# natir/yacrd

Hardware: AMD Instinct MI355X
Metric: reads_per_sec_classified (higher is better)
Workload: dtype u32

## Files before the change

yacrd_amd/csrc/screen_reg.h:

```cpp
#pragma once
#include "device_common.h"
#include "wave_ops.h"

namespace yk {

#ifndef YK_SCREEN_WINDOW
#define YK_SCREEN_WINDOW 32
#endif
constexpr int kScreenWindow = YK_SCREEN_WINDOW;
constexpr int kScreenTabWords = (64 / 16) * (16 + 2 * kScreenWindow) * 4;
template <int WPB, int WORDS = kScreenTabWords>
__device__ __forceinline__ u32 *wave_screen_scratch()
{
    __shared__ __attribute__((aligned(16))) u32 s_tab[WPB][WORDS];
    return s_tab[threadIdx.x >> 6];
}

template <int LANES>
__device__ __forceinline__ bool group_any(u64 ballot)
{
    if (LANES == 64) return ballot != 0;
    return ((u32)(ballot >> (lane_id() & (u32)(64 - LANES))) & (u32)((1ull << (LANES & 63)) - 1ull)) != 0u;
}

struct HealthyRead {
    u32 a, b;
    i32 F, G;
};
#ifndef YK_SCREEN_SLIDES
#define YK_SCREEN_SLIDES 4
#endif
constexpr int kScreenSlides = YK_SCREEN_SLIDES;

template <int LANES, int WPB, bool SLID = false, int TABW = kScreenTabWords>
__device__ __forceinline__ bool healthy_screen(const uint4 (&v)[4], const bool (&real0)[4], const bool (&real1)[4],
                                               u32 len, i32 c, u32 pmin, u32 pmax, HealthyRead &hr, u32 P = 0, u32 Q = 0,
                                               u32 emin = 0, u32 smax = 0xFFFFFFFFu)
{
    constexpr int NB = LANES, W = kScreenWindow, NBIN = 2 * W + NB, GROUPS = 64 / LANES, PER = W / LANES,
                  ZPER = NBIN / LANES;
    constexpr u32 kEnd = 1u << 10, kField = kEnd - 1u;
    static_assert(W % LANES == 0 && PER >= 1 && W <= 64, "window bins per lane; a window index has six bits");
    static_assert(NBIN % LANES == 0 && GROUPS * NBIN * 4 <= TABW, "scratch");
    const u32 lane = lane_id(), lig = lane & (u32)(LANES - 1), grp = lane / (u32)LANES;
    u32 *tab = wave_screen_scratch<WPB, TABW>() + grp * (u32)(NBIN * 4);
    uint4 *bins = reinterpret_cast<uint4 *>(tab);
    char *tb = reinterpret_cast<char *>(tab);

    const i32 bits = 32 - (i32)__builtin_clz(len | 1u) - ilog2c(NB) + (len != 0 ? 0 : -1);
    const u32 sh = (u32)max(bits, ilog2c(W));
    const u32 span = pmax - pmin, T = span - (u32)W;

#pragma unroll
    for (int q = 0; q < ZPER; q++) bins[lig + (u32)(LANES * q)] = make_uint4(0u, 0u, 0u, 0u);
    wave_lds_sync();

    const u32 cp = (lig & 3u) * 4u;
    u32 one = 1u, one_end = kEnd;
    if constexpr (!SLID) asm volatile("" : "+v"(one), "+v"(one_end));
    u32 ramp = 0;
    auto count = [&](u32 s, u32 e, bool real) {
        const u32 ds = s - pmin, dx = e - pmin;
        const u32 is = min(ds, (u32)W) + (ds >> sh);
        const u32 ie = (dx >> sh) + __builtin_elementwise_sub_sat(dx, T) + (u32)W;
        if constexpr (SLID) {
            const bool in_ramp = ds >= (u32)W && s < emin;
            ramp += (real && s >= pmin && in_ramp) ? 1u : 0u;
            if (real && s >= pmin && !in_ramp) atomicAdd(reinterpret_cast<u32 *>(tb + ((is << 4) + cp)), one);
            if (real && e <= pmax && !(e > smax && dx <= T)) atomicAdd(reinterpret_cast<u32 *>(tb + ((ie << 4) + cp)), one_end);
        } else if (real) {
            atomicAdd(reinterpret_cast<u32 *>(tb + ((is << 4) + cp)), one);
            atomicAdd(reinterpret_cast<u32 *>(tb + ((ie << 4) + cp)), one_end);
        }
    };
#pragma unroll
    for (int j = 0; j < 4; j++) {
        count(v[j].x, v[j].y, real0[j]);
        count(v[j].z, v[j].w, real1[j]);
    }
    wave_lds_sync();

    u32 f[PER], fw = 0;
#pragma unroll
    for (int q = 0; q < PER; q++) {
        const u32 d = lig * (u32)PER + q;
        const u32 it = min((u32)(2 * W) - d + ((span - d) >> sh), (u32)(NBIN - 1));
        const uint4 h4 = bins[d], t4 = bins[it];
        f[q] = ((h4.x + h4.y + h4.z + h4.w) & kField) | ((t4.x + t4.y + t4.z + t4.w) & (kField << 10));
        fw += f[q];
    }
    const uint4 c4 = bins[(u32)W + lig];
    const u32 fincl = gscan_add<LANES>(fw);
    u32 reached = 0;
    {
        const u32 k1 = (u32)min(c + 1, 0x1FF);
        u32 run = fincl - fw + (SLID ? ((512u - k1 + P) | ((512u - k1 + Q) << 10)) : (512u - k1) * (1u | kEnd));
#pragma unroll
        for (int q = 0; q < PER; q++) {
            run += f[q];
            reached += run & (0x200u | (0x200u << 10));
        }
    }
    const u32 cand = (((u32)PER - ((reached >> 9) & 7u)) << 20) | (((u32)PER - (reached >> 19)) << 26);
    const u32 w = (c4.x + c4.y + c4.z + c4.w) & ((kField << 10) | kField);
    const u32 wincl = gscan_add<LANES>(w | cand);
    const u32 ex = wincl - w;
    const i32 x = (i32)(ex & kField) - (i32)((wincl >> 10) & kField);
    const u32 xm = gscan_min<LANES>((w & kField) != 0u ? (u32)(x + 0x10000) : 0xFFFFFFFFu);
    const i32 F = (i32)(fincl & kField) + (SLID ? (i32)P : 0), G = (i32)(fincl >> 10) + (SLID ? (i32)Q : 0);
    hr.F = F, hr.G = G;
    hr.a = pmin + ((wincl >> 20) & 63u);
    hr.b = pmax - (wincl >> 26);
    i32 open0 = F;
    if constexpr (SLID) open0 += (i32)gscan_add<LANES>(ramp);
    const bool deep = xm == 0xFFFFFFFFu || (i32)(xm - 0x10000u) + open0 > c;
    return deep && F > c && G > c;
}

struct VerdictsToGlobal {
    const SweepArgs &a;
    __device__ __forceinline__ void closed(u32 r, u32 ra, u32 rb, u32 len) const
    {
        if (ra != 0 || rb != len) a.closed[r] = make_uint2(ra, rb);
        else a.counts[r] = 0;
        if (a.prefilter == 2) atomicAdd(&a.ctr->prefiltered, 1u);
    }
    __device__ __forceinline__ void deferred(u32 r) const { a.counts[r] = kDeferredMark; }
};

template <int ITEMS>
struct ReadsKnown {
    u64 o[ITEMS];
    u32 n[ITEMS], len[ITEMS];
};

template <int LANES, int ITEMS, bool WIDE, int WPB = 1, class Sink>
__device__ __forceinline__ void screen_reads(const SweepArgs &a, const u32 (&r)[ITEMS], const bool (&active)[ITEMS], const Sink &sink,
                                             const ReadsKnown<ITEMS> *known = nullptr)
{
    constexpr int K = 16;
    const u32 lane = lane_id(), lig = lane & (u32)(LANES - 1);
    const i32 c = (i32)min(a.cov, 0x3FFFFFFFu);
    u32 n[ITEMS], len[ITEMS];
    u64 o[ITEMS];
#pragma unroll
    for (int t = 0; t < ITEMS; t++) {
        o[t] = 0, n[t] = 0, len[t] = 0;
        if (known) {
            if (active[t]) o[t] = known->o[t], n[t] = known->n[t], len[t] = known->len[t];
        } else if (active[t]) {
            const ulonglong2 oo = load_extent(a.off + r[t]);
            o[t] = oo.x;
            n[t] = (u32)(oo.y - oo.x);
            len[t] = a.len[r[t]];
        }
    }
    uint4 v[ITEMS][K / 4];
#pragma unroll
    for (int t = 0; t < ITEMS; t++) {
        const bool two = n[t] >= 2u;
        const uint2 *src = two ? a.iv + o[t] : reinterpret_cast<const uint2 *>(a.off);
        const u32 last2 = two ? n[t] - 2u : 0u;
#pragma unroll
        for (int j = 0; j < K / 4; j++)
            v[t][j] = load_pair<(ITEMS >= 2)>(src + min(2u * (lig + (u32)LANES * j), last2));
    }
#pragma unroll
    for (int t = 0; t < ITEMS; t++) {
        if (t > 0 && __builtin_amdgcn_ballot_w64(active[t]) == 0) break;
        const u32 len_c = min(len[t], kMaxKeyPos);
        u32 smin = v[t][0].x, emax = v[t][0].y, smax = v[t][0].x;
        i32 tmin = 0x7FFFFFFF;
#pragma unroll
        for (int j = 0; j < K / 4; j++) {
            smin = min(smin, min(v[t][j].x, v[t][j].z));
            smax = max(smax, max(v[t][j].x, v[t][j].z));
            emax = max(emax, max(v[t][j].y, v[t][j].w));
            tmin = min(tmin, min((i32)(v[t][j].y - v[t][j].x), (i32)(v[t][j].w - v[t][j].z)));
        }
        const int last_addr = (int)((lane | (u32)(LANES - 1)) << 2);
        const u32 pmin = (u32)__builtin_amdgcn_ds_bpermute(last_addr, (int)gscan_min<LANES>(smin));
        const u32 pmax = (u32)__builtin_amdgcn_ds_bpermute(last_addr, (int)gscan_max<LANES>(emax));
        const bool irregular = n[t] < 2u || pmax > len_c || smax > kMaxKeyPos || tmin < (i32)kScreenWindow;
        const bool girr = group_any<LANES>(__builtin_amdgcn_ballot_w64(irregular));
        const u32 n_eff = girr ? 0u : n[t];
        bool real0[K / 4], real1[K / 4];
#pragma unroll
        for (int j = 0; j < K / 4; j++) {
            const u32 i0 = 2u * (lig + (u32)LANES * j);
            real0[j] = i0 + 1u < n_eff;
            real1[j] = i0 < n_eff;
        }
        HealthyRead hr;
        bool healthy = healthy_screen<LANES, WPB, false, kScreenTabWords>(v[t], real0, real1, len[t], c, pmin, pmax, hr) && !girr;
        if constexpr (kScreenSlides > 0 && WIDE) {
            auto state_of = [&](bool nd, const HealthyRead &h) {
                return (nd ? 1u : 0u) | ((u32)min(max(h.F, 0), 1023) << 1) | ((u32)min(max(h.G, 0), 1023) << 11);
            };
            u32 st = state_of(!healthy && !girr && (i32)n[t] > c && (hr.F <= 3 * c + 6 || hr.G <= c), hr);
            if (__builtin_amdgcn_ballot_w64((st & 1u) != 0 && lig == (u32)(LANES - 1)) != 0) {
                u32 emin = v[t][0].y, smax2 = v[t][0].x;
#pragma unroll
                for (int j = 0; j < K / 4; j++) {
                    emin = min(emin, min(v[t][j].y, v[t][j].w));
                    smax2 = max(smax2, max(v[t][j].x, v[t][j].z));
                }
                const u32 gemin = (u32)__builtin_amdgcn_ds_bpermute(last_addr, (int)gscan_min<LANES>(emin));
                const u32 room_h = gemin - pmin;
                const u32 gsmax = (u32)__builtin_amdgcn_ds_bpermute(last_addr, (int)gscan_max<LANES>(smax2));
                const u32 room_t = pmax - gsmax;
                u32 ht = 0, PQ = 0;
#pragma unroll 1
                for (int slide = 0; slide < kScreenSlides; slide++) {
                    const u32 g = (u32)__builtin_amdgcn_ds_bpermute(last_addr, (int)st);
                    const bool gneed = (g & 1u) != 0;
                    const u32 gF = (g >> 1) & 1023u, gG = g >> 11;
                    if (gneed && (i32)gF <= c) ht += (u32)kScreenWindow, PQ = (PQ & 0xFFFF0000u) | gF;
                    if (gneed && (i32)gG <= c) ht += (u32)kScreenWindow << 16, PQ = (PQ & 0xFFFFu) | (gG << 16);
                    const u32 h0 = ht & 0xFFFFu, t0 = ht >> 16;
                    const bool go = gneed && room_h >= h0 + (u32)kScreenWindow && room_t >= t0 + (u32)kScreenWindow &&
                                    pmax - pmin >= h0 + t0 + 2u * (u32)kScreenWindow;
                    if (__builtin_amdgcn_ballot_w64(go) == 0) break;
                    bool r0[K / 4], r1[K / 4];
#pragma unroll
                    for (int j = 0; j < K / 4; j++) r0[j] = real0[j] && go, r1[j] = real1[j] && go;
                    wave_lds_sync();
                    HealthyRead h2;
                    const bool ok2 = healthy_screen<LANES, WPB, true, kScreenTabWords>(v[t], r0, r1, len[t], c, pmin + h0, pmax - t0, h2, PQ & 0xFFFFu, PQ >> 16, gemin, gsmax);
                    st = go ? state_of(!ok2 && (h2.F <= c || h2.G <= c), h2) : 0u;
                    if (go) healthy = ok2, hr.a = h2.a, hr.b = h2.b, hr.F = h2.F, hr.G = h2.G;
                }
            }
        }
        if (lig == (u32)(LANES - 1) && active[t]) {
            if (healthy || (!girr && (i32)n[t] <= c)) {
                const u32 ra = (i32)n[t] <= c ? len[t] : hr.a, rb = (i32)n[t] <= c ? len[t] : hr.b;
                sink.closed(r[t], ra, rb, len[t]);
            } else {
                sink.deferred(r[t]);
            }
        }
        if (t + 1 < ITEMS) wave_lds_sync();
    }
}

template <int LANES, int ITEMS, bool WIDE = false>
__device__ __forceinline__ void screen_block(const SweepArgs &a, u32 block)
{
    constexpr u32 GROUPS = 64 / LANES;
    const u32 grp = lane_id() / (u32)LANES;
    const u32 list_n = *a.list_n;
    const u32 idx0 = a.first + block * (u32)ITEMS * GROUPS;
    if (idx0 >= list_n) return;
    u32 r[ITEMS];
    bool active[ITEMS];
#pragma unroll
    for (int t = 0; t < ITEMS; t++) {
        const u32 idx = idx0 + (u32)t * GROUPS + grp;
        active[t] = idx < list_n;
        r[t] = active[t] ? a.list[idx] : 0u;
    }
    screen_reads<LANES, ITEMS, WIDE>(a, r, active, VerdictsToGlobal{a});
}

}
```

yacrd_amd/csrc/sweep_wave.h:

```cpp
#pragma once
#include <type_traits>

#include "device_common.h"
#include "screen_reg.h"
#include "wave_ops.h"

namespace yk {

constexpr u32 kPadKey = 0xFFFFFFFEu;

template <int LANES, int K>
__device__ __forceinline__ void sweep_group_keys(u32 (&x)[K], u32 m, u32 len, i32 c,
                                                 bool active, u32 r, u64 badmask, u64 zmask,
                                                 bool zl_check, const SweepArgs &a,
                                                 const LaneConst &lc)
{
    const u32 lane = lane_id(), lig = lane & (u32)(LANES - 1);
    auto slot_of = [&]() {
        u32 rr = r;
        asm volatile("" : "+v"(rr));
        return a.stage + (a.off[rr] + 2 * (u64)rr);
    };

    bitonic_sort<LANES, K, 2>(x, lc);

    if (zl_check) {
        bool dup = false;
#pragma unroll
        for (int q = 0; q + 1 < K; q++) dup |= x[q] == x[q + 1] && (x[q] & 3u) == 1u && x[q] != 1u;
        const u32 prev = gshift_up1<LANES>(x[K - 1]);
        dup |= lig != 0 && prev == x[0] && (prev & 3u) == 1u && prev != 1u;
        badmask |= __builtin_amdgcn_ballot_w64(dup);
    }
    const bool group_bad = LANES == 64   ? badmask != 0
                           : LANES == 32 ? (u32)(badmask >> (lane & 32u)) != 0
                                         : ((u32)(badmask >> (lane & 48u)) & 0xFFFFu) != 0;

    u32 n_starts = 0;
#pragma unroll
    for (int q = 0; q < K; q++) n_starts += x[q] & 1u;
    const u32 delta = 2u * n_starts - (u32)K;
    const u32 dincl = gscan_add<LANES>(delta);
    const i32 depth_in = (i32)(dincl - delta);

    const u32 tail_base = m - lig * (u32)K;
    const u32 len_key = len > kMaxKeyPos ? 0xFFFFFFFFu : (len << kKeyShift);
    u32 mf_incl, ml_incl, mf_in, ml_in;
    u32 cnt = 0, fb = 0, fe = 0, cand = kNoKey;
    auto passes = [&](auto zl_tag) {
        constexpr bool ZL = decltype(zl_tag)::value;
        u32 mf = 0, ml = 0;
        i32 dd = depth_in;
#pragma unroll
        for (int q = 0; q < K; q++) {
            const u32 key = x[q], bit = key & 1u;
            const bool is_s = bit != 0, gt = dd > c + q;
            ml = (is_s && !gt) ? key : ml;
            if (ZL) mf = (!is_s && gt) ? max(mf, key ^ 2u) : mf;
            else mf = (!is_s && gt) ? key : mf;
            dd += (i32)(bit << 1);
        }
        if (!ZL) mf = mf ? (mf ^ 2u) : 0u;
        mf_incl = gscan_max<LANES>(mf);
        ml_incl = gscan_max<LANES>(ml);
        mf_in = max(gshift_up1<LANES>(mf_incl), kNoFlag);
        ml_in = gshift_up1<LANES>(ml_incl);

        u32 tc = ZL ? mf_in : (mf_in ^ 2u);
        u32 cml = ml_in;
        dd = depth_in;
#pragma unroll
        for (int q = 0; q < K; q++) {
            const u32 key = x[q], bit = key & 1u;
            const bool is_s = bit != 0, gt = dd > c + q;
            const bool fl = !is_s && gt, low = is_s && !gt;
            const bool eff = ZL ? (fl && (key ^ 2u) > tc) : fl;
            const u32 begin = ZL ? (tc ^ 2u) : tc;
            const bool close = eff && cml > begin;
            cnt += close ? 1u : 0u;
            fb = close ? begin : fb;
            fe = close ? cml : fe;
            const bool tail = fl && ((u32)dd == tail_base) && key >= len_key;
            cand = min(cand, tail ? (key >> kKeyShift) : kNoKey);
            tc = eff ? (ZL ? (key ^ 2u) : key) : tc;
            cml = low ? key : cml;
            dd += (i32)(bit << 1);
        }
    };
    if (zmask == 0) passes(std::false_type{});
    else passes(std::true_type{});
    i32 d;

    const bool live = active && !group_bad;
    u32 g_closed = 0;
    if (__builtin_amdgcn_ballot_w64(cnt != 0) != 0) {
        const u32 cincl = gscan_add<LANES>(cnt);
        g_closed = cincl;
        u32 pos = cincl - cnt;
        if (live && cnt == 1) {
            slot_of()[pos] = make_uint2(fb >> kKeyShift, fe >> kKeyShift);
        } else if (live && cnt > 1) {
            uint2 *slot = slot_of();
            u32 tc = mf_in, cml = ml_in;
            d = depth_in;
#pragma unroll
            for (int q = 0; q < K; q++) {
                const u32 key = x[q];
                const bool is_s = (key & 1u) != 0, gt = d > c;
                const bool fl = !is_s && gt, low = is_s && !gt;
                const bool eff = fl && (key ^ 2u) > tc;
                if (eff && cml > (tc ^ 2u))
                    slot[pos++] = make_uint2((tc ^ 2u) >> kKeyShift, cml >> kKeyShift);
                tc = eff ? (key ^ 2u) : tc;
                cml = low ? key : cml;
                d += is_s ? 1 : -1;
            }
        }
    }
    u32 min_ge = kNoKey;
    if (__builtin_amdgcn_ballot_w64(cand != kNoKey) != 0) min_ge = gscan_min<LANES>(cand);
    if (lig == LANES - 1 && active) {
        if (group_bad) {
            a.rej_list[atomicAdd(a.rej_count, 1u)] = r;
            a.counts[r] = 0;
        } else {
            a.counts[r] = finish_read(slot_of(), g_closed, mf_incl ? (mf_incl ^ 2u) : 0u, ml_incl, min_ge, len);
        }
    }
}


constexpr int kFilterTabWords = 304, kFilterKeyWords = 512;
template <int WPB>
__device__ __forceinline__ u32 *wave_filter_scratch()
{
    __shared__ __attribute__((aligned(16))) u32 s_scratch[WPB][kFilterTabWords + kFilterKeyWords];
    return s_scratch[threadIdx.x >> 6];
}

template <int LANES, int K, int WPB>
__device__ __forceinline__ bool prefilter(const u32 (&x)[K], u32 n, u32 len, i32 c, u32 (&y)[K / 2],
                                          u32 &m_out)
{
    static_assert(K == 16, "a lane reads its K/2 = 8 compacted keys as two 16-byte vectors");
    constexpr int NB = LANES, CAP = LANES * K / 2, GROUPS = 64 / LANES;
    static_assert(GROUPS * (NB + 1) * 4 <= kFilterTabWords && GROUPS * CAP <= kFilterKeyWords, "scratch");
    const u32 lane = lane_id(), lig = lane & (u32)(LANES - 1), grp = lane / (u32)LANES;
    u32 *scratch = wave_filter_scratch<WPB>();
    u32 *tab = scratch + grp * (u32)((NB + 1) * 4);
    u32 *keys = scratch + kFilterTabWords + grp * (u32)CAP;
    uint4 *my_bin = reinterpret_cast<uint4 *>(tab) + lig;
    uint4 *my_keys = reinterpret_cast<uint4 *>(keys) + lig * 2u;

    const i32 bits = 32 - (i32)__builtin_clz(len | 1u) - ilog2c(NB) + (len != 0 ? 0 : -1);
    const u32 sh = (u32)max(bits, 0), ksh = sh + kKeyShift;

    *my_bin = make_uint4(0u, 0u, 0u, 0u);
    my_keys[0] = make_uint4(kPadKey, kPadKey, kPadKey, kPadKey);
    my_keys[1] = make_uint4(kPadKey, kPadKey, kPadKey, kPadKey);
    wave_lds_sync();
    u32 *cell0 = tab + (lig & 3u);
    u32 *pad_cell = cell0 + NB * 4;
    u32 *cell[K];
#pragma unroll
    for (int q = 0; q < K; q++) {
        const bool real = lig + (u32)LANES * (q / 2) < n;
        u32 *p = cell0 + (x[q] >> ksh) * 4u;
        cell[q] = real ? p : pad_cell;
        atomicAdd(cell[q], (q & 1) ? 0x10000u : 1u);
    }
    wave_lds_sync();
    const uint4 w4 = *my_bin;
    const u32 w = w4.x + w4.y + w4.z + w4.w;
    const u32 incl = gscan_add<LANES>(w);
    const i32 S = (i32)(w & 0xFFFFu), E = (i32)(w >> 16);
    const i32 cs = (i32)(incl & 0xFFFFu), ce = (i32)(incl >> 16);
    const i32 depth_after = cs - ce, depth_at = depth_after - (S - E);
    const bool safe = (cs - S) - ce > c && lig < (len >> sh);
    const u64 sball = __builtin_amdgcn_ballot_w64(safe);
    if (sball == 0) return false;
    const u64 smask = LANES == 64 ? sball
                                  : (sball >> (lane & (u32)(64 - LANES))) & ((1ull << (LANES & 63)) - 1ull);
    const bool head = safe && (((smask << 1) >> lig) & 1ull) == 0;
    const bool tail = safe && (((smask >> 1) >> lig) & 1ull) == 0;
    const u32 hv = gscan_max<LANES>(head ? (((lig + 1u) << 16) | (u32)depth_at) : 0u);
    const i32 net = tail ? depth_after - (i32)(hv & 0xFFFFu) : 0;
    const u32 nsyn = min((u32)(net < 0 ? -net : net), (u32)CAP + 1u);
    const u32 synkey = (((hv >> 16) - 1u) << ksh) | (net > 0 ? 3u : 0u);

    const u32 mine = safe ? nsyn : (u32)(S + E);
    const u32 rincl = gscan_add<LANES>(mine);
    const u32 m = (u32)__builtin_amdgcn_ds_bpermute((int)((lane | (u32)(LANES - 1)) << 2), (int)rincl);
    if (__builtin_amdgcn_ballot_w64(m > (u32)CAP) != 0) return false;
    const u32 base = rincl - mine;
    {
        uint4 b4;
        b4.x = base;
        b4.y = b4.x + (w4.x & 0xFFFFu) + (w4.x >> 16);
        b4.z = b4.y + (w4.y & 0xFFFFu) + (w4.y >> 16);
        b4.w = b4.z + (w4.z & 0xFFFFu) + (w4.z >> 16);
        *my_bin = safe ? make_uint4(CAP, CAP, CAP, CAP) : b4;
        if (lig < 4u) tab[NB * 4 + lig] = (u32)CAP;
    }
#pragma unroll 1
    for (u32 t = 0; t < nsyn; t++) keys[base + t] = synkey;
    wave_lds_sync();
#pragma unroll
    for (int q0 = 0; q0 < K; q0 += 8) {
        u32 pos[8];
#pragma unroll
        for (int q = 0; q < 8; q++) pos[q] = atomicAdd(cell[q0 + q], 1u);
#pragma unroll
        for (int q = 0; q < 8; q++) {
            if (pos[q] < (u32)CAP) keys[pos[q]] = x[q0 + q];
        }
    }
    wave_lds_sync();
    const uint4 lo = my_keys[0], hi = my_keys[1];
    y[0] = lo.x, y[1] = lo.y, y[2] = lo.z, y[3] = lo.w;
    y[4] = hi.x, y[5] = hi.y, y[6] = hi.z, y[7] = hi.w;
    m_out = m;
    return true;
}

template <int LANES, int K, int WPB = 4>
__device__ __forceinline__ void sweep_group_read(const uint2 *__restrict__ iv, u32 n, u32 len,
                                                 u32 cov, bool active, u32 r,
                                                 const SweepArgs &a, const LaneConst &lc)
{
    const u32 lane = lane_id(), lig = lane & (u32)(LANES - 1);
    const i32 c = (i32)min(cov, 0x3FFFFFFFu);

    u32 x[K];
    u32 bad = 0, nz = 0;
    bool plain;
    {
        const uint2 *src = n ? iv : reinterpret_cast<const uint2 *>(a.off);
        const u32 last = n ? n - 1u : 0u;
        uint2 v[K / 2];
#pragma unroll
        for (int j = 0; j < K / 2; j++) v[j] = src[min(lig + (u32)LANES * j, last)];
        const u32 len_c = min(len, kMaxKeyPos);
        u32 irregular = 0;
#pragma unroll
        for (int j = 0; j < K / 2; j++) {
            const bool real = lig + (u32)LANES * j < n;
            irregular |= (real && (v[j].x >= v[j].y || v[j].y > len_c)) ? 1u : 0u;
            x[2 * j] = real ? ((v[j].x << kKeyShift) | 3u) : kPadKey;
            x[2 * j + 1] = real ? (v[j].y << kKeyShift) : kPadKey;
        }
        plain = __builtin_amdgcn_ballot_w64(irregular != 0) == 0;
        if (!plain) {
#pragma unroll
            for (int j = 0; j < K / 2; j++) {
                u32 ks, ke, b = 0, z = 0;
                make_event_keys(v[j], ks, ke, b, z);
                const bool real = lig + (u32)LANES * j < n;
                x[2 * j] = real ? ks : kPadKey;
                x[2 * j + 1] = real ? ke : kPadKey;
                bad |= real ? b : 0u;
                nz += real ? z : 0u;
            }
        }
    }
    const u64 badmask = __builtin_amdgcn_ballot_w64(bad != 0);
    const u64 zmask = __builtin_amdgcn_ballot_w64(nz != 0);
    if (LANES == 64 && badmask != 0) {
        if (lig == LANES - 1 && active) {
            a.rej_list[atomicAdd(a.rej_count, 1u)] = r;
            a.counts[r] = 0;
        }
        return;
    }
    const bool zl_check = (zmask & (zmask - 1)) != 0 || __builtin_amdgcn_ballot_w64(nz > 2) != 0;

    if constexpr (K == 16) {
        if (a.prefilter && plain) {
            u32 y[K / 2], mf;
            if (prefilter<LANES, K, WPB>(x, n, len, c, y, mf)) {
                if (a.prefilter == 2 && lig == 0 && active) atomicAdd(&a.ctr->prefiltered, 1u);
                sweep_group_keys<LANES, K / 2>(y, mf, len, c, active, r, badmask, zmask, zl_check, a, lc);
                return;
            }
        }
    }
    sweep_group_keys<LANES, K>(x, 2 * n, len, c, active, r, badmask, zmask, zl_check, a, lc);
}

template <int LANES, int K, int WPB = 4>
__device__ __forceinline__ void sweep_group_block(const SweepArgs &a, u32 block)
{
    const u32 lane = lane_id();
    const LaneConst lc = make_lane_const(lane);

    constexpr u32 GROUPS = 64 / LANES;
    const u32 list_n = *a.list_n;
    const u32 wave = block * (u32)WPB + (threadIdx.x >> 6);
    if (a.first + wave * GROUPS >= list_n) return;
    const u32 idx = a.first + wave * GROUPS + lane / (u32)LANES;
    const bool active = idx < list_n;
    u32 r = 0, n = 0, len = 0;
    u64 o = 0;
    if (active) {
        r = a.list[idx];
        o = a.off[r];
        n = (u32)(a.off[r + 1] - o);
        len = a.len[r];
    }
    sweep_group_read<LANES, K, WPB>(a.iv + o, n, len, a.cov, active, r, a, lc);
}

template <int LANES, int K>
__global__ __launch_bounds__(256) void sweep_group_kernel(SweepArgs a)
{
    sweep_group_block<LANES, K>(a, blockIdx.x);
}

template <int LANES, int K>
inline void launch_sweep_group(const SweepArgs &sa, u32 n_reads, hipStream_t stream)
{
    constexpr u32 per_block = 4u * (64 / LANES);
    const u32 grid = (n_reads + per_block - 1) / per_block;
    hipLaunchKernelGGL((sweep_group_kernel<LANES, K>), dim3(grid ? grid : 1), dim3(256), 0, stream, sa);
}

#ifndef YK_DEFER_OCC
#define YK_DEFER_OCC 6
#endif
constexpr int kFusedWaves = 4, kDeferWaves = 1, kDeferOcc = YK_DEFER_OCC;
static_assert(kDeferWaves == 1, "screen_block indexes list entries by workgroup: one wavefront each");
struct FusedArgs {
    SweepArgs base;
    u32 n_entries;
    u32 cls[5];
    u32 block_end[5];
    u32 first[5];
    const u32 *list[5];
    const u32 *list_n[5];
};

template <bool DEFER, int WPB, int ITEMS = 1, bool WIDE = false>
__device__ __forceinline__ void sweep_small_fused_body(const FusedArgs &f)
{
    u32 g = blockIdx.x;
    {
        const u32 nb = gridDim.x, x = g & 7u, q = nb >> 3, rem = nb & 7u;
        g = x * q + min(x, rem) + (g >> 3);
    }
    u32 e = 0, first = 0;
    while (e + 1 < f.n_entries && g >= f.block_end[e]) {
        first = f.block_end[e];
        e++;
    }
    SweepArgs a = f.base;
    a.list = f.list[e];
    a.list_n = f.list_n[e];
    a.first = f.first[e];
    const u32 b = g - first;
    switch (f.cls[e]) {
    case CLS_R2: sweep_group_block<16, 2, WPB>(a, b); break;
    case CLS_R4: sweep_group_block<16, 4, WPB>(a, b); break;
    case CLS_R8: sweep_group_block<16, 8, WPB>(a, b); break;
    case CLS_R16:
        if constexpr (DEFER) screen_block<16, ITEMS, WIDE>(a, b);
        else sweep_group_block<16, 16, WPB>(a, b);
        break;
    default:
        if constexpr (DEFER) screen_block<32, ITEMS, WIDE>(a, b);
        else sweep_group_block<32, 16, WPB>(a, b);
        break;
    }
}
__global__ __launch_bounds__(64 * kDeferWaves, kDeferOcc) void sweep_small_fused_defer_kernel(FusedArgs f)
{
    sweep_small_fused_body<true, kDeferWaves>(f);
}
__global__ __launch_bounds__(64 * kDeferWaves, kDeferOcc) void sweep_small_fused_defer_wide_kernel(FusedArgs f)
{
    sweep_small_fused_body<true, kDeferWaves, 1, true>(f);
}
#ifndef YK_DEFER2_OCC
#define YK_DEFER2_OCC YK_DEFER_OCC
#endif
__global__ __launch_bounds__(64, YK_DEFER2_OCC) void sweep_small_fused_defer2_kernel(FusedArgs f)
{
    sweep_small_fused_body<true, 1, 2>(f);
}
__global__ __launch_bounds__(64 * kFusedWaves, 5) void sweep_small_fused_kernel(FusedArgs f)
{
    sweep_small_fused_body<false, kFusedWaves>(f);
}

inline u32 sweep_group_reads_per_block(int cls, int waves = 4)
{
    return ((cls <= CLS_R16) ? 4u : (cls == CLS_H16) ? 2u : 1u) * (u32)waves;
}

}
```

Measured before the change: 2.921 billion.

## Screen 32-interval reads with 16-lane groups holding two bins per lane

Makes healthy_screen generic in bin count and interval pairs per lane, so a 16-lane group can cover 32 bins with two bins per lane and scan over them locally. In the defer2 (two-item, non-wide) kernel, the default-class reads now go through 16-lane groups processing one read with K=32 intervals, instead of 32-lane groups with two items. The scratch table grows to fit the larger bin count. The aim is to screen four reads per wave instead of two. The cost is more per-lane work, more registers and more LDS per wave.

```diff
diff --git a/yacrd_amd/csrc/screen_reg.h b/yacrd_amd/csrc/screen_reg.h
--- a/yacrd_amd/csrc/screen_reg.h
+++ b/yacrd_amd/csrc/screen_reg.h
@@ -9,6 +9,7 @@
 #endif
 constexpr int kScreenWindow = YK_SCREEN_WINDOW;
 constexpr int kScreenTabWords = (64 / 16) * (16 + 2 * kScreenWindow) * 4;
+constexpr int kScreenTabWordsRows = (64 / 16) * (32 + 2 * kScreenWindow) * 4;
 template <int WPB, int WORDS = kScreenTabWords>
 __device__ __forceinline__ u32 *wave_screen_scratch()
 {
@@ -32,16 +33,17 @@
 #endif
 constexpr int kScreenSlides = YK_SCREEN_SLIDES;
 
-template <int LANES, int WPB, bool SLID = false, int TABW = kScreenTabWords>
-__device__ __forceinline__ bool healthy_screen(const uint4 (&v)[4], const bool (&real0)[4], const bool (&real1)[4],
+template <int LANES, int WPB, bool SLID = false, int TABW = kScreenTabWords, int NB = LANES, int PAIRS = 4>
+__device__ __forceinline__ bool healthy_screen(const uint4 (&v)[PAIRS], const bool (&real0)[PAIRS], const bool (&real1)[PAIRS],
                                                u32 len, i32 c, u32 pmin, u32 pmax, HealthyRead &hr, u32 P = 0, u32 Q = 0,
                                                u32 emin = 0, u32 smax = 0xFFFFFFFFu)
 {
-    constexpr int NB = LANES, W = kScreenWindow, NBIN = 2 * W + NB, GROUPS = 64 / LANES, PER = W / LANES,
-                  ZPER = NBIN / LANES;
+    constexpr int W = kScreenWindow, NBIN = 2 * W + NB, GROUPS = 64 / LANES, PER = W / LANES, ZPER = NBIN / LANES,
+                  CPL = NB / LANES;
     constexpr u32 kEnd = 1u << 10, kField = kEnd - 1u;
     static_assert(W % LANES == 0 && PER >= 1 && W <= 64, "window bins per lane; a window index has six bits");
-    static_assert(NBIN % LANES == 0 && GROUPS * NBIN * 4 <= TABW, "scratch");
+    static_assert(NB % LANES == 0 && NBIN % LANES == 0 && GROUPS * NBIN * 4 <= TABW, "scratch");
+    static_assert(PAIRS * 2 * LANES <= 256, "a counter field has ten bits");
     const u32 lane = lane_id(), lig = lane & (u32)(LANES - 1), grp = lane / (u32)LANES;
     u32 *tab = wave_screen_scratch<WPB, TABW>() + grp * (u32)(NBIN * 4);
     uint4 *bins = reinterpret_cast<uint4 *>(tab);
@@ -74,7 +76,7 @@
         }
     };
 #pragma unroll
-    for (int j = 0; j < 4; j++) {
+    for (int j = 0; j < PAIRS; j++) {
         count(v[j].x, v[j].y, real0[j]);
         count(v[j].z, v[j].w, real1[j]);
     }
@@ -89,7 +91,13 @@
         f[q] = ((h4.x + h4.y + h4.z + h4.w) & kField) | ((t4.x + t4.y + t4.z + t4.w) & (kField << 10));
         fw += f[q];
     }
-    const uint4 c4 = bins[(u32)W + lig];
+    u32 wb[CPL], w = 0;
+#pragma unroll
+    for (int q = 0; q < CPL; q++) {
+        const uint4 c4 = bins[(u32)W + lig * (u32)CPL + q];
+        wb[q] = (c4.x + c4.y + c4.z + c4.w) & ((kField << 10) | kField);
+        w += wb[q];
+    }
     const u32 fincl = gscan_add<LANES>(fw);
     u32 reached = 0;
     {
@@ -102,11 +110,16 @@
         }
     }
     const u32 cand = (((u32)PER - ((reached >> 9) & 7u)) << 20) | (((u32)PER - (reached >> 19)) << 26);
-    const u32 w = (c4.x + c4.y + c4.z + c4.w) & ((kField << 10) | kField);
     const u32 wincl = gscan_add<LANES>(w | cand);
-    const u32 ex = wincl - w;
-    const i32 x = (i32)(ex & kField) - (i32)((wincl >> 10) & kField);
-    const u32 xm = gscan_min<LANES>((w & kField) != 0u ? (u32)(x + 0x10000) : 0xFFFFFFFFu);
+    u32 run = wincl - w, xl = 0xFFFFFFFFu;
+#pragma unroll
+    for (int q = 0; q < CPL; q++) {
+        const u32 ex = run;
+        run += wb[q];
+        const i32 x = (i32)(ex & kField) - (i32)((run >> 10) & kField);
+        xl = min(xl, (wb[q] & kField) != 0u ? (u32)(x + 0x10000) : 0xFFFFFFFFu);
+    }
+    const u32 xm = gscan_min<LANES>(xl);
     const i32 F = (i32)(fincl & kField) + (SLID ? (i32)P : 0), G = (i32)(fincl >> 10) + (SLID ? (i32)Q : 0);
     hr.F = F, hr.G = G;
     hr.a = pmin + ((wincl >> 20) & 63u);
@@ -134,11 +147,12 @@
     u32 n[ITEMS], len[ITEMS];
 };
 
-template <int LANES, int ITEMS, bool WIDE, int WPB = 1, class Sink>
+template <int LANES, int ITEMS, bool WIDE, int WPB = 1, int K = 16, int NB = LANES, bool NT = (ITEMS >= 2),
+          int TABW = kScreenTabWords, class Sink>
 __device__ __forceinline__ void screen_reads(const SweepArgs &a, const u32 (&r)[ITEMS], const bool (&active)[ITEMS], const Sink &sink,
                                              const ReadsKnown<ITEMS> *known = nullptr)
 {
-    constexpr int K = 16;
+    static_assert(K % 4 == 0, "a lane takes its intervals in pairs");
     const u32 lane = lane_id(), lig = lane & (u32)(LANES - 1);
     const i32 c = (i32)min(a.cov, 0x3FFFFFFFu);
     u32 n[ITEMS], len[ITEMS];
@@ -163,7 +177,7 @@
         const u32 last2 = two ? n[t] - 2u : 0u;
 #pragma unroll
         for (int j = 0; j < K / 4; j++)
-            v[t][j] = load_pair<(ITEMS >= 2)>(src + min(2u * (lig + (u32)LANES * j), last2));
+            v[t][j] = load_pair<NT>(src + min(2u * (lig + (u32)LANES * j), last2));
     }
 #pragma unroll
     for (int t = 0; t < ITEMS; t++) {
@@ -192,7 +206,7 @@
             real1[j] = i0 < n_eff;
         }
         HealthyRead hr;
-        bool healthy = healthy_screen<LANES, WPB, false, kScreenTabWords>(v[t], real0, real1, len[t], c, pmin, pmax, hr) && !girr;
+        bool healthy = healthy_screen<LANES, WPB, false, TABW, NB>(v[t], real0, real1, len[t], c, pmin, pmax, hr) && !girr;
         if constexpr (kScreenSlides > 0 && WIDE) {
             auto state_of = [&](bool nd, const HealthyRead &h) {
                 return (nd ? 1u : 0u) | ((u32)min(max(h.F, 0), 1023) << 1) | ((u32)min(max(h.G, 0), 1023) << 11);
@@ -226,7 +240,7 @@
                     for (int j = 0; j < K / 4; j++) r0[j] = real0[j] && go, r1[j] = real1[j] && go;
                     wave_lds_sync();
                     HealthyRead h2;
-                    const bool ok2 = healthy_screen<LANES, WPB, true, kScreenTabWords>(v[t], r0, r1, len[t], c, pmin + h0, pmax - t0, h2, PQ & 0xFFFFu, PQ >> 16, gemin, gsmax);
+                    const bool ok2 = healthy_screen<LANES, WPB, true, TABW, NB>(v[t], r0, r1, len[t], c, pmin + h0, pmax - t0, h2, PQ & 0xFFFFu, PQ >> 16, gemin, gsmax);
                     st = go ? state_of(!ok2 && (h2.F <= c || h2.G <= c), h2) : 0u;
                     if (go) healthy = ok2, hr.a = h2.a, hr.b = h2.b, hr.F = h2.F, hr.G = h2.G;
                 }
@@ -244,7 +258,7 @@
     }
 }
 
-template <int LANES, int ITEMS, bool WIDE = false>
+template <int LANES, int ITEMS, bool WIDE = false, int K = 16, int NB = LANES, bool NT = (ITEMS >= 2), int TABW = kScreenTabWords>
 __device__ __forceinline__ void screen_block(const SweepArgs &a, u32 block)
 {
     constexpr u32 GROUPS = 64 / LANES;
@@ -260,7 +274,7 @@
         active[t] = idx < list_n;
         r[t] = active[t] ? a.list[idx] : 0u;
     }
-    screen_reads<LANES, ITEMS, WIDE>(a, r, active, VerdictsToGlobal{a});
-}
-
-}
+    screen_reads<LANES, ITEMS, WIDE, 1, K, NB, NT, TABW>(a, r, active, VerdictsToGlobal{a});
+}
+
+}
diff --git a/yacrd_amd/csrc/sweep_wave.h b/yacrd_amd/csrc/sweep_wave.h
--- a/yacrd_amd/csrc/sweep_wave.h
+++ b/yacrd_amd/csrc/sweep_wave.h
@@ -357,16 +357,19 @@
     a.list_n = f.list_n[e];
     a.first = f.first[e];
     const u32 b = g - first;
+    constexpr bool ROWS = DEFER && ITEMS == 2 && !WIDE;
+    constexpr int TABW = ROWS ? kScreenTabWordsRows : kScreenTabWords;
     switch (f.cls[e]) {
     case CLS_R2: sweep_group_block<16, 2, WPB>(a, b); break;
     case CLS_R4: sweep_group_block<16, 4, WPB>(a, b); break;
     case CLS_R8: sweep_group_block<16, 8, WPB>(a, b); break;
     case CLS_R16:
-        if constexpr (DEFER) screen_block<16, ITEMS, WIDE>(a, b);
+        if constexpr (DEFER) screen_block<16, ITEMS, WIDE, 16, 16, (ITEMS >= 2), TABW>(a, b);
         else sweep_group_block<16, 16, WPB>(a, b);
         break;
     default:
-        if constexpr (DEFER) screen_block<32, ITEMS, WIDE>(a, b);
+        if constexpr (ROWS) screen_block<16, 1, false, 32, 32, true, TABW>(a, b);
+        else if constexpr (DEFER) screen_block<32, ITEMS, WIDE>(a, b);
         else sweep_group_block<32, 16, WPB>(a, b);
         break;
     }
```

Result: faster. 3.117 billion, median of 6 (+6.7%).
